# bluenote-1577/sylph

Hardware: AMD Instinct MI355X
Metric: read Gbp/s sketched + genome-comparisons/s profiled, 1 Gbp vs GTDB-R220 (higher is better)
Workload: dtype u64

## Files before the change

sylph_amd/csrc/common.h:

```cpp
#pragma once
#include <hip/hip_runtime.h>

#include <atomic>
#include <cstdarg>
#include <cstdint>
#include <cstdio>
#include <cstdlib>
#include <cstring>
#include <ctime>
#include <map>
#include <mutex>
#include <string>
#include <vector>

#include "../../include/sylph_hip.h"

struct sylph_ctx;

namespace sylph {

void set_error(const char* fmt, ...);

struct HipError { hipError_t e; const char* what; const char* file; int line; };

// ... 134 lines not shown
    sylph::DevBuf scratch[8];
    sylph::DevBuf counters;
    void* pinned = nullptr;
    void read_back(void* dst, const void* dev_src, size_t bytes);
    static constexpr size_t STAGE_BYTES = 32u << 20;
    void* stage[2] = {nullptr, nullptr};
    hipEvent_t stage_ev[2] = {nullptr, nullptr};
    hipStream_t copy_stream = nullptr;
    hipEvent_t copy_ev[2] = {nullptr, nullptr};
    void d2h(void* dst, const void* dev_src, size_t bytes);
    void h2d(void* dev_dst, const void* src, size_t bytes);
};

namespace sylph {

struct ScopedKernelTimer {
    sylph_ctx* ctx;
    hipEvent_t a = nullptr, b = nullptr;
    const char* fam;
    ScopedKernelTimer(sylph_ctx* c, const char* family);
    ~ScopedKernelTimer();
};
void profile_collect(sylph_ctx* ctx);
void ctx_unref(sylph_ctx* ctx);

struct HostPhase {
    sylph_ctx* ctx;
    const char* name;
    double t0 = 0;
    static bool enabled() { static const bool e = getenv("SYLPH_HIP_TRACE") != nullptr; return e; }
    static double now() { timespec ts; clock_gettime(CLOCK_MONOTONIC, &ts); return ts.tv_sec * 1e3 + ts.tv_nsec * 1e-6; }
    HostPhase(sylph_ctx* c, const char* n) : ctx(c), name(n) { if (enabled()) { (void)hipStreamSynchronize(c->stream); t0 = now(); } }
    ~HostPhase() { if (enabled()) { (void)hipStreamSynchronize(ctx->stream); fprintf(stderr, "[sylph_hip] %-28s %8.3f ms\n", name, now() - t0); } }
};

struct DeviceGuard {
    int prev = -1;
    explicit DeviceGuard(int dev) {
        (void)hipGetDevice(&prev);
        if (prev != dev) SY_HIP(hipSetDevice(dev));
        else prev = -1;
    }
    ~DeviceGuard() { if (prev >= 0) (void)hipSetDevice(prev); }
};

void sort_pairs_u64_u32(sylph_ctx* ctx, const uint64_t* kin, uint64_t* kout, const uint32_t* vin, uint32_t* vout,
                        size_t n, int begin_bit, int end_bit);
void sort_pairs_u32_u64(sylph_ctx* ctx, const uint32_t* kin, uint32_t* kout, const uint64_t* vin, uint64_t* vout,
                        size_t n, int begin_bit, int end_bit);
void sort_pairs_u32_u32(sylph_ctx* ctx, const uint32_t* kin, uint32_t* kout, const uint32_t* vin, uint32_t* vout,
                        size_t n, int begin_bit, int end_bit);
constexpr uint32_t SPILL_MAX_TILES = 256;
struct SpillState { uint32_t n_tiles; uint32_t tiles[SPILL_MAX_TILES]; };
struct ReadsState { uint32_t long_record; SpillState spill; };

void sort_keys_u32(sylph_ctx* ctx, const uint32_t* kin, uint32_t* kout, size_t n, int begin_bit, int end_bit);
void sort_keys_u64(sylph_ctx* ctx, const uint64_t* kin, uint64_t* kout, size_t n, int begin_bit, int end_bit);
void exclusive_sum_u32(sylph_ctx* ctx, const uint32_t* in, uint32_t* out, size_t n);
void inclusive_max_u32(sylph_ctx* ctx, const uint32_t* in, uint32_t* out, size_t n);

inline int bit_length(uint64_t v) { int b = 0; while (v) { b++; v >>= 1; } return b; }

}
```

sylph_amd/csrc/reads.hip:

```cpp
#include <cstddef>

#include "common.h"
#include "device_common.h"
#include "sketch_session.h"

namespace sylph {

namespace {

constexpr int RTPB = 256;
constexpr int RT_MIN = 4096, RT_MAX = 65536;
constexpr int RH = 400;
constexpr int RPAD = 32;
constexpr int MASKW = 12;
constexpr int OFFS_256 = 600;
constexpr int RTPB_RAGGED = 512;

template <int K>
struct KC {
    static constexpr uint64_t MASK = (1ull << (2 * K)) - 1;
};

__device__ __forceinline__ uint64_t win64(const uint32_t* sF, uint32_t b) {
    const uint32_t j = b >> 4, ph = (b & 15u) * 2u;
    const uint64_t x = ((uint64_t)sF[j] << 32) | sF[j + 1];
    return (x << ph) | ((uint64_t)sF[j + 2] >> (32u - ph));
}

template <int K>
__device__ __forceinline__ uint64_t revcomp_top(uint64_t x) {
    const uint64_t rev = __brevll(x);
    const uint64_t y = ((rev & 0x5555555555555555ull) << 1) | ((rev >> 1) & 0x5555555555555555ull);
    return (~y) & KC<K>::MASK;
}

__device__ __forceinline__ uint32_t even_fields_to_bytes31(uint32_t w) {
    uint32_t t = w & 0xCCCCCCCCu;
    t = (t | (t << 2)) & 0xF0F0F0F0u;
    return t | (t << 4);
}
__device__ __forceinline__ void evenodd16(uint64_t x, uint32_t& ev, uint32_t& od) {
    const uint32_t hi = (uint32_t)(x >> 32), lo = (uint32_t)x;
    ev = __builtin_amdgcn_perm(even_fields_to_bytes31(hi), even_fields_to_bytes31(lo), 0x07050301u);
    od = __builtin_amdgcn_perm(even_fields_to_bytes31(hi << 2), even_fields_to_bytes31(lo << 2), 0x07050301u);
}

template <int K, int T, int HV>
__device__ __forceinline__ void kmer_step(uint32_t A0, uint32_t A1, uint32_t A2, uint32_t Bm, uint32_t B0, uint32_t B1, uint32_t B2,
                                          uint64_t thr, uint32_t& mask) {
    constexpr int D = 64 - 2 * K;
    uint32_t fhi, flo, rhi, rlo;
    if constexpr (T == 0) { fhi = A0; flo = A1; }
    else { fhi = __builtin_amdgcn_alignbit(A0, A1, 32 - 2 * T); flo = __builtin_amdgcn_alignbit(A1, A2, 32 - 2 * T); }
    constexpr int OFF = 2 * T - D;
    if constexpr (OFF < 0) { rlo = __builtin_amdgcn_alignbit(B0, Bm, OFF + 32); rhi = __builtin_amdgcn_alignbit(B1, B0, OFF + 32); }
    else if constexpr (OFF == 0) { rlo = B0; rhi = B1; }
    else { rlo = __builtin_amdgcn_alignbit(B1, B0, OFF); rhi = __builtin_amdgcn_alignbit(B2, B1, OFF); }
    const uint64_t f = ((uint64_t)fhi << 32) | flo, rc = ((uint64_t)rhi << 32) | rlo;
    const uint64_t canon = (f < rc ? f : rc) >> D;
    if constexpr (HV == 2) {
        const uint32_t u = mm_hash64_gfx950_hi1(canon);
        asm("v_cmp_ge_u32 vcc, %2, %1\n\tv_addc_co_u32 %0, vcc, %0, %0, vcc" : "+v"(mask) : "v"(u), "s"((uint32_t)thr) : "vcc");
    } else {
        const uint64_t h = HV ? mm_hash64_gfx950(canon) : mm_hash64(canon);
        asm("v_cmp_lt_u64 vcc, %1, %2\n\tv_addc_co_u32 %0, vcc, %0, %0, vcc" : "+v"(mask) : "v"(h), "s"(thr) : "vcc");
    }
}
template <int K, int T0, int HV>
__device__ __forceinline__ void kmer_steps8(uint32_t A0, uint32_t A1, uint32_t A2, uint32_t Bm, uint32_t B0, uint32_t B1, uint32_t B2,
                                            uint64_t thr, uint32_t& mask) {
    kmer_step<K, T0 + 0, HV>(A0, A1, A2, Bm, B0, B1, B2, thr, mask);
    kmer_step<K, T0 + 1, HV>(A0, A1, A2, Bm, B0, B1, B2, thr, mask);
    kmer_step<K, T0 + 2, HV>(A0, A1, A2, Bm, B0, B1, B2, thr, mask);
    kmer_step<K, T0 + 3, HV>(A0, A1, A2, Bm, B0, B1, B2, thr, mask);
    kmer_step<K, T0 + 4, HV>(A0, A1, A2, Bm, B0, B1, B2, thr, mask);
    kmer_step<K, T0 + 5, HV>(A0, A1, A2, Bm, B0, B1, B2, thr, mask);
    kmer_step<K, T0 + 6, HV>(A0, A1, A2, Bm, B0, B1, B2, thr, mask);
    kmer_step<K, T0 + 7, HV>(A0, A1, A2, Bm, B0, B1, B2, thr, mask);
}

__global__ __launch_bounds__(256) void block_records_kernel(const uint64_t* __restrict__ off, uint64_t n_rec, uint32_t bias,
                                                            uint32_t rt, uint32_t n_entries, uint32_t* __restrict__ blk_rec,
                                                            uint32_t* __restrict__ count_sentinel, uint32_t* __restrict__ state_words) {
    const uint32_t b = blockIdx.x * blockDim.x + threadIdx.x;
    if (b == 0) { *count_sentinel = 0; state_words[0] = 0; state_words[1] = 0; }
    if (b >= n_entries) return;
    const uint64_t target = (uint64_t)b * rt;
    uint64_t lo = 0, hi = n_rec;
    while (lo < hi) {
        const uint64_t mid = (lo + hi) >> 1;
        if (off[mid] + bias < target) lo = mid + 1; else hi = mid;
    }
    blk_rec[b] = (uint32_t)lo;
}

#ifndef SYLPH_READS_HASH_DEFAULT
#define SYLPH_READS_HASH_DEFAULT 1
#endif
#ifndef SYLPH_READS_WAVES
#define SYLPH_READS_WAVES 5
#endif
template <int K, int HV, int ENC, int TPB>
__global__ __launch_bounds__(TPB) __attribute__((amdgpu_waves_per_eu(TPB == 256 ? SYLPH_READS_WAVES : 6, TPB == 256 ? SYLPH_READS_WAVES : 6))) void reads_kernel(const uint8_t* __restrict__ bases_al, uint32_t bias, uint64_t n_al,
                                                     const uint64_t* __restrict__ off, uint64_t n_rec,
                                                     const uint32_t* __restrict__ blk_rec, uint32_t n_blk, uint32_t it_begin, uint32_t it_end,
                                                     uint32_t rt, uint64_t thr,
                                                     uint32_t cand_slack, int avx2_compat, int paired, int want_markers, uint64_t rec_base,
                                                     uint32_t slot_cap, OccRec* __restrict__ slot_rec,
                                                     uint32_t* __restrict__ slot_key, int key_sh,
                                                     uint32_t* __restrict__ blk_count,
                                                     ReadsState* __restrict__ state, const uint32_t* __restrict__ blk_list,
                                                     uint32_t* __restrict__ spill_slot_of_blk) {
    constexpr int RTPB = TPB, OFFS = TPB == 256 ? OFFS_256 : 2 * TPB + 80;
    extern __shared__ uint32_t sF[];
    __shared__ uint64_t s_off[OFFS + 4];
    const uint32_t n_words = (rt + 2 * RH) / 16 + 3;
    __shared__ uint32_t s_mask[MASKW][RTPB];
    __shared__ uint32_t s_wave[RTPB / 64];
    static_assert((OFFS + 4) >= 2 * RTPB, "the marker arrays alias the staged offsets");
    uint64_t* const s_m0 = s_off;
    uint64_t* const s_m1 = s_off + RTPB;
    __shared__ uint32_t s_first[RTPB + 1], s_rel[RTPB];
    __shared__ uint16_t s_perm[RTPB], s_nh[RTPB];
    const uint32_t tid = threadIdx.x, lane = tid & 63, wave = tid >> 6;
    __shared__ uint32_t s_redo, s_redo_deal;
    const uint64_t thr_loop = HV == 2 ? (uint64_t)((uint32_t)(thr >> 32) + 1u + cand_slack) : thr;
    if (tid == 0) s_redo = 0;
    const uint32_t per_xcd = (n_blk + 7) / 8;
    for (uint32_t it0 = it_begin + blockIdx.x; it0 < it_end; it0 += gridDim.x) {
        const uint32_t it = blk_list ? it0 : (it0 & 7u) * per_xcd + (it0 >> 3);
        if (it >= n_blk) continue;
        const uint32_t blk = blk_list ? blk_list[it] : it;
        const int64_t a0 = (int64_t)blk * rt - RH;
        const bool interior = a0 >= 0 && (uint64_t)(a0 + (int64_t)n_words * 16) <= n_al;
        if (interior) {
            if constexpr (ENC == 0) {
                const uint4* __restrict__ src = reinterpret_cast<const uint4*>(bases_al + a0);
                for (uint32_t ci = tid; ci < n_words; ci += RTPB) sF[ci] = pack16_fwd(src[ci]);
            } else {
                const uint32_t* __restrict__ src = reinterpret_cast<const uint32_t*>(bases_al + (a0 >> 2));
                for (uint32_t ci = tid; ci < n_words; ci += RTPB) sF[ci] = __builtin_amdgcn_perm(0u, src[ci], 0x00010203u);
            }
        } else {
            for (uint32_t ci = tid; ci < n_words; ci += RTPB) {
                const int64_t a = a0 + (int64_t)ci * 16;
                if constexpr (ENC == 0) {
                    uint4 v = make_uint4(0, 0, 0, 0);
                    if (a >= 0 && (uint64_t)a < n_al) v = *reinterpret_cast<const uint4*>(bases_al + a);
                    sF[ci] = pack16_fwd(v);
                } else {
                    uint32_t w = 0;
                    if (a >= 0 && (uint64_t)a < n_al) w = *reinterpret_cast<const uint32_t*>(bases_al + (a >> 2));
                    sF[ci] = __builtin_amdgcn_perm(0u, w, 0x00010203u);
                }
            }
        }
        const uint64_t R0 = blk_rec[blk], R1 = blk_rec[blk + 1];
        const uint64_t w_lo = paired ? (R0 & ~1ull) : R0;
        const uint64_t w_hi = min(R1 + 2, n_rec);
        const bool in_lds = (w_hi - w_lo + 1) <= (uint64_t)(OFFS + 4) && (R1 - R0) <= (uint64_t)RTPB;
        if (in_lds)
            for (uint64_t t = tid; t <= w_hi - w_lo; t += RTPB) s_off[t] = off[w_lo + t];
        __syncthreads();
        uint32_t base_prev = 0;
        const uint64_t out0 = (uint64_t)it * slot_cap;
        for (uint64_t pass = R0; pass < R1; pass += RTPB) {
            const uint64_t r = pass + tid;
            const bool active = r < R1;
            uint64_t start = 0, L = 0, s1 = 0, s2 = 0, e2 = 0;
            if (active) {
                if (in_lds) {
                    start = s_off[r - w_lo];
                    L = s_off[r + 1 - w_lo] - start;
                    if (paired) { const uint64_t r1 = (r & ~1ull) - w_lo; s1 = s_off[r1]; s2 = s_off[r1 + 1]; e2 = s_off[r1 + 2]; }
                } else {
                    start = off[r];
                    L = off[r + 1] - start;
                    if (paired) { const uint64_t r1 = r & ~1ull; s1 = off[r1]; s2 = off[r1 + 1]; e2 = off[r1 + 2]; }
                }
            }
            const bool too_long = active && (L > (uint64_t)RH || (paired && (s2 - s1 > (uint64_t)RH || e2 - s2 > (uint64_t)RH)));
            if (too_long) state->long_record = 1u;
            const uint32_t nh = (active && !too_long) ? (uint32_t)n_hashed_kmers(L, K, avx2_compat, 0) : 0u;
            const uint32_t rel = active ? (uint32_t)((int64_t)(start + bias) - a0) : 0u;
            uint32_t* const s_hist = s_first;
            if (tid < 64) s_hist[tid] = 0;
            s_rel[tid] = rel;
            s_nh[tid] = (uint16_t)nh;
#ifndef SYLPH_READS_ALWAYS_DEAL
            if (tid == 0) s_redo_deal = 0;
            __syncthreads();
            if (__ballot(nh != (uint32_t)s_nh[0]) && lane == 0) s_redo_deal = 1;
            __syncthreads();
            const bool dealt = s_redo_deal != 0;
            const uint32_t bin = 63u - ((nh + 7) >> 3);
            uint32_t hg_max = (nh + 7) >> 3, arrival = 0, hc = 0;
            if (dealt) {
                arrival = atomicAdd(&s_hist[bin], 1u);
                __syncthreads();
                hc = s_hist[lane];
                const uint64_t bins_used = __ballot(hc != 0u);
                hg_max = bins_used ? 63u - (uint32_t)(__ffsll((unsigned long long)bins_used) - 1) : 0u;
            }
#else
            __syncthreads();
            const uint32_t bin = 63u - ((nh + 7) >> 3);
            const uint32_t arrival = atomicAdd(&s_hist[bin], 1u);
            __syncthreads();
            const uint32_t hc = s_hist[lane];
            const bool dealt = s_hist[bin] != (uint32_t)RTPB;
            const uint64_t bins_used = __ballot(hc != 0u);
            const uint32_t hg_max = bins_used ? 63u - (uint32_t)(__ffsll((unsigned long long)bins_used) - 1) : 0u;
#endif
            const uint32_t rows_used = min((uint32_t)MASKW, (hg_max * 8u + 31u) >> 5);
            if (dealt) {
                const uint32_t incl = wave_inclusive_sum(hc);
                s_perm[(uint32_t)__shfl((int)(incl - hc), (int)bin) + arrival] = (uint16_t)tid;
                __syncthreads();
            }
            const uint32_t slot = dealt ? s_perm[tid] : tid;
            const uint32_t rel_h = dealt ? s_rel[slot] : rel, nh_h = dealt ? s_nh[slot] : nh;
            uint32_t nh_max = nh_h;
#pragma unroll
            for (int d = 32; d > 0; d >>= 1) nh_max = max(nh_max, (uint32_t)__shfl_xor((int)nh_max, d));
            if (nh_max) {
                const uint32_t w0 = rel_h >> 4, sh = 32u - (rel_h & 15u) * 2u;
                uint32_t raw = sF[w0], nxt = sF[w0 + 1];
                auto next_word = [&](uint32_t j) {
                    const uint32_t a = (uint32_t)((((uint64_t)raw << 32) | nxt) >> sh);
                    raw = nxt;
                    nxt = sF[w0 + j + 2];
                    return a;
                };
                uint32_t A0 = next_word(0), A1 = next_word(1), A2 = next_word(2);
                uint32_t Bm = 0, B0 = rcword(A0), B1 = rcword(A1), B2 = rcword(A2);
                const uint32_t n_half = (nh_max + 7) >> 3;
// ... 174 lines not shown
__global__ __launch_bounds__(1024) void block_total_kernel(const uint32_t* __restrict__ blk_count, uint32_t n_blk, uint32_t* __restrict__ total) {
    __shared__ uint32_t s[16];
    uint32_t v = 0;
    for (uint32_t i = threadIdx.x; i < n_blk; i += 1024) v += blk_count[i];
#pragma unroll
    for (int d = 32; d > 0; d >>= 1) v += (uint32_t)__shfl_xor((int)v, d);
    if ((threadIdx.x & 63) == 0) s[threadIdx.x >> 6] = v;
    __syncthreads();
    if (threadIdx.x == 0) {
        uint32_t t = 0;
        for (int w = 0; w < 16; w++) t += s[w];
        *total = t;
    }
}

struct SlotMeta {
    uint32_t *blk_rec, *blk_count, *spill_slot, *blk_off;
    ReadsState* state;
    SlotMeta(sylph_sketch* sk, uint32_t n_blk) {
        blk_rec = sk->slot_meta.as<uint32_t>();
        blk_count = blk_rec + (n_blk + 1);
        spill_slot = blk_count + (n_blk + 1);
        blk_off = spill_slot + (n_blk + 1);
        state = reinterpret_cast<ReadsState*>(blk_off + (n_blk + 1));
    }
};

void compact_region(sylph_sketch* sk, uint32_t n_blk, uint32_t slot_cap, uint32_t n, uint32_t spill_cap, const OccRec* spill_rec) {
    sylph_ctx* ctx = sk->ctx;
    SlotMeta m(sk, n_blk);
    exclusive_sum_u32(ctx, m.blk_count, m.blk_off, (size_t)n_blk + 1);
    const uint64_t need = sk->n_occ + n;
    sk->hash.grow_keep(need * 8, sk->n_occ * 8, ctx->stream);
    sk->recs.grow_keep(need * sizeof(OccRec), sk->n_occ * sizeof(OccRec), ctx->stream);
    {
        ScopedKernelTimer t(ctx, "compact");
        hipLaunchKernelGGL(compact_occ_kernel, dim3(std::min<uint32_t>(n_blk, 1u << 16)), dim3(64), 0, ctx->stream,
                           sk->slot_rec.as<OccRec>(), m.blk_count, m.blk_off, n_blk, slot_cap, spill_cap, spill_rec, m.spill_slot,
                           sk->hash.as<uint64_t>() + sk->n_occ, sk->recs.as<OccRec>() + sk->n_occ);
        SY_HIP(hipGetLastError());
    }
    sk->n_occ = need;
}

}

void resolve_deferred_slots(sylph_sketch* sk) {
    if (!sk->pend.live || !sk->pend.deferred) return;
    sylph_ctx* ctx = sk->ctx;
    SlotMeta m(sk, sk->pend.n_blk);
    hipLaunchKernelGGL(block_total_kernel, dim3(1), dim3(1024), 0, ctx->stream, m.blk_count, sk->pend.n_blk, m.blk_off + sk->pend.n_blk);
    uint32_t res[3] = {0, 0, 0};
    ctx->read_back(res, m.blk_off + sk->pend.n_blk, 12);
    if (res[1] || res[2]) { redo_deferred_batch(sk); return; }
    sk->pend.deferred = false;
    sk->pend.n = res[0];
    if (res[0] == 0) sk->pend = PendingSlots{};
}

void flush_pending_slots(sylph_sketch* sk) {
    resolve_deferred_slots(sk);
    if (!sk->pend.live) return;
    compact_region(sk, sk->pend.n_blk, sk->pend.slot_cap, sk->pend.n, 0, nullptr);
    sk->pend = PendingSlots{};
}

bool push_short_reads(sylph_sketch* sk, const uint8_t* d_bases, uint32_t phase, const uint64_t* d_off, uint64_t n_records, uint64_t n_bases,
                      int enc) {
    sylph_ctx* ctx = sk->ctx;
    const uint32_t bias = enc == SYLPH_ENC_2BIT ? (uint32_t)((uintptr_t)d_bases & 15) * 4u + phase : (uint32_t)((uintptr_t)d_bases & 15);
    const uint8_t* bases_al = d_bases - ((uintptr_t)d_bases & 15);
    const uint64_t n_al = n_bases + bias;
    static const int env_ragged_tpb = [] { const char* e = getenv("SYLPH_HIP_READS_RAGGED_TPB"); return e ? atoi(e) : RTPB; }();
    const bool ragged = (n_bases % n_records) != 0;
    const int tpb = (ragged && env_ragged_tpb == RTPB_RAGGED && (uint64_t)RTPB_RAGGED * 93 / 100 * n_bases / n_records <= (uint64_t)RT_MAX) ? RTPB_RAGGED : RTPB;
    const uint64_t target = ragged ? (uint64_t)tpb * 93 / 100 : (uint64_t)tpb;
    uint32_t rt = (uint32_t)std::min<uint64_t>(RT_MAX, std::max<uint64_t>(RT_MIN, target * n_bases / n_records));
    rt = (rt + 15u) & ~15u;
    const uint32_t n_blk = (uint32_t)(n_al / rt) + 1;
    const uint64_t expect = (uint64_t)rt / sk->c;
    const uint32_t spill_cap = rt + RH;
    const uint32_t slot_cap = (uint32_t)std::min<uint64_t>(spill_cap, expect + expect * 3 / 4 + 48);
    const size_t lds_bytes = ((size_t)(rt + 2 * RH) / 16 + 3 + RPAD) * 4;
    const uint64_t thr = UINT64_MAX / (uint64_t)sk->c;
    sk->slot_rec.reserve((size_t)n_blk * slot_cap * sizeof(OccRec));
    sk->slot_key.reserve((size_t)n_blk * slot_cap * 4);
    sk->slot_meta.reserve(((size_t)n_blk + 1) * 4 * 4 + sizeof(ReadsState) + 16);
    SlotMeta m(sk, n_blk);
    static_assert(offsetof(ReadsState, long_record) == 0 && offsetof(ReadsState, spill) == 4 && offsetof(SpillState, n_tiles) == 0,
                  "long_record and spill.n_tiles are the first two words");
    int cus = 256;
    (void)hipDeviceGetAttribute(&cus, hipDeviceAttributeMultiprocessorCount, ctx->device);
    static const int hv_env = getenv("SYLPH_HIP_HASH_VARIANT") ? atoi(getenv("SYLPH_HIP_HASH_VARIANT")) : SYLPH_READS_HASH_DEFAULT;
    const int hv_want = ctx->reads_hash >= 0 ? ctx->reads_hash : hv_env;
    const uint32_t slack = ctx->reads_slack;
    const int hv = (hv_want == 2 && ((thr >> 32) + 1ull + slack) > 0xFFFFFFFFull) ? 1 : hv_want;
    const int key_sh = key_shift(sk->c);
    auto launch = [&](uint32_t n_it, uint32_t it_b, uint32_t it_e, uint32_t cap, OccRec* sr, uint32_t* skey, const uint32_t* list) {
        if (it_e <= it_b) return;
        const uint32_t grid = ctx->reads_wg_per_cu ? (uint32_t)std::min<uint64_t>(it_e - it_b, (uint64_t)cus * ctx->reads_wg_per_cu) : it_e - it_b;
#define SY_LAUNCH_READS_T(KK, HH, EE, TT)                                                                                             \
    hipLaunchKernelGGL((reads_kernel<KK, HH, EE, TT>), dim3(grid), dim3(TT), lds_bytes, ctx->stream, bases_al, bias, n_al, d_off, n_records, \
                       m.blk_rec, n_it, it_b, it_e, rt, thr, slack, sk->avx2_compat, sk->paired, sk->no_dedup ? 0 : 1, sk->rec_base, cap, sr, skey, key_sh,   \
                       m.blk_count, m.state, list, m.spill_slot)
#define SY_LAUNCH_READS(KK, HH, EE) do { if (tpb == RTPB_RAGGED) SY_LAUNCH_READS_T(KK, HH, EE, RTPB_RAGGED); else SY_LAUNCH_READS_T(KK, HH, EE, RTPB); } while (0)
        if (enc == SYLPH_ENC_2BIT) {
            if (sk->k == 31) { if (hv == 2) SY_LAUNCH_READS(31, 2, 1); else SY_LAUNCH_READS(31, 1, 1); }
            else { if (hv == 2) SY_LAUNCH_READS(21, 2, 1); else SY_LAUNCH_READS(21, 1, 1); }
        } else if (sk->k == 31) { if (hv == 2) SY_LAUNCH_READS(31, 2, 0); else if (hv) SY_LAUNCH_READS(31, 1, 0); else SY_LAUNCH_READS(31, 0, 0); }
        else { if (hv == 2) SY_LAUNCH_READS(21, 2, 0); else if (hv) SY_LAUNCH_READS(21, 1, 0); else SY_LAUNCH_READS(21, 0, 0); }
#undef SY_LAUNCH_READS_T
#undef SY_LAUNCH_READS
        SY_HIP(hipGetLastError());
    };
    {
        HostPhase ph(ctx, "push: reads kernel");
        {
            ScopedKernelTimer t(ctx, "annotate");
            hipLaunchKernelGGL(block_records_kernel, dim3(grid_for(n_blk + 1)), dim3(256), 0, ctx->stream, d_off, n_records, bias, rt,
                               n_blk + 1, m.blk_rec, m.blk_count + n_blk, reinterpret_cast<uint32_t*>(m.state));
        }
        ctx->seed_gate();
        {
            const uint32_t n_round = ((n_blk + 7) / 8) * 8;
            uint32_t cut = n_round;
            if (ctx->turn.done && !ctx->turn.recorded && ctx->reads_tail_pct && n_round >= 64)
                cut = (uint32_t)((uint64_t)n_round * (100 - ctx->reads_tail_pct) / 100) & ~7u;
            {
                ScopedKernelTimer t(ctx, "seeds");
                launch(n_blk, 0, cut, slot_cap, sk->slot_rec.as<OccRec>(), sk->slot_key.as<uint32_t>(), nullptr);
            }
            ctx->seed_done();
            if (cut < n_round) {
                ScopedKernelTimer t(ctx, "seeds");
                launch(n_blk, cut, n_round, slot_cap, sk->slot_rec.as<OccRec>(), sk->slot_key.as<uint32_t>(), nullptr);
            }
        }
        const uint64_t n_expect = (n_bases > n_records * (uint64_t)(sk->k - 1) ? n_bases - n_records * (uint64_t)(sk->k - 1) : 0) / sk->c;
        if (sk->borrow_until_finish && sk->n_occ == 0 && sk->rec_base == 0 && ctx->finish_mode == 0 && sk->c >= 2 && n_expect >= 4096 &&
            (uint64_t)n_blk * slot_cap < (1ull << 31)) {
            sk->pend = PendingSlots{};
            sk->pend.live = true;
            sk->pend.deferred = true;
            sk->pend.n_blk = n_blk;
            sk->pend.slot_cap = slot_cap;
            sk->pend.n = n_blk * slot_cap;
            sk->pend.n_expect = (uint32_t)std::min<uint64_t>(n_expect, sk->pend.n);
            sk->pend.bases = d_bases; sk->pend.phase = phase; sk->pend.off = d_off;
            sk->pend.n_records = n_records; sk->pend.n_bases = n_bases; sk->pend.enc = enc;
            if (ctx->profile) ctx->stats["deferred"].launches++;
            return true;
        }
        hipLaunchKernelGGL(block_total_kernel, dim3(1), dim3(1024), 0, ctx->stream, m.blk_count, n_blk, m.blk_off + n_blk);
    }
    uint32_t res[3] = {0, 0, 0};
    SY_HIP(hipMemcpyAsync(ctx->pinned, m.blk_off + n_blk, 12, hipMemcpyDeviceToHost, ctx->stream));
    SY_HIP(hipStreamSynchronize(ctx->stream));
    memcpy(res, ctx->pinned, 12);
    if (!ctx->pending.empty()) profile_collect(ctx);
    if (res[1] || res[2] > SPILL_MAX_TILES) return false;
    const uint32_t n = res[0];
    if (n == 0) return true;
    if (res[2] == 0 && sk->n_occ == 0 && ctx->finish_mode != 1 && sk->c >= 2) {
        sk->pend.live = true;
        sk->pend.n_blk = n_blk;
        sk->pend.slot_cap = slot_cap;
        sk->pend.n = n;
        return true;
    }
    const OccRec* sp_r = nullptr;
    if (res[2]) {
        DevBuf& b_x = ctx->scratch[7];
        b_x.reserve((size_t)res[2] * spill_cap * sizeof(OccRec));
        OccRec* xr = b_x.as<OccRec>();
        ScopedKernelTimer ts(ctx, "seeds_spill");
        ScopedKernelTimer t(ctx, "seeds");
        launch(res[2], 0, res[2], spill_cap, xr, nullptr, m.state->spill.tiles);
        sp_r = xr;
    }
    compact_region(sk, n_blk, slot_cap, n, spill_cap, sp_r);
    return true;
}

}
```

sylph_amd/csrc/replay_lds.hip:

```cpp
#include "common.h"
#include "device_common.h"
#include "sketch_session.h"
#include "partition.h"

namespace sylph {
namespace {

#ifndef SYLPH_REPLAY_TPB
#define SYLPH_REPLAY_TPB 128
#endif
constexpr int CAP_SMALL = 256, RTPB_SMALL = SYLPH_REPLAY_TPB;
constexpr int CAP_MID = 512, RTPB_MID = 256;
constexpr int CAP_LARGE = 1024, RTPB_LARGE = 256;
constexpr int IDX_BITS = 10;
constexpr uint32_t SEG_LIMIT = 96;


struct ReplayArgs {
    const OccRec* recs;
    const uint64_t* hash;
    const uint32_t* perm;
    const uint32_t* boff;
    const uint32_t* p_nv;
    int paired, dedup;
// ... 877 lines not shown
    uint32_t* chunk_rows = mid_list + (B + 2) + ((B & 1u) ? 1 : 0);
    unsigned long long* chunk_removed = reinterpret_cast<unsigned long long*>(chunk_rows + 264);
    FinishTail* d_tail = b_small.as<FinishTail>();
    const uint32_t* d_nv = boff + B;
    const uint32_t n_zero = (B + 2) * 2;
    const int dbg = getenv("SYLPH_REPLAY_STAGE") ? atoi(getenv("SYLPH_REPLAY_STAGE")) : 0;
    const uint32_t cutoff = sk->paired ? 0u : 4u;
    sk->out_k.reserve((size_t)n_cap * 8);
    sk->out_c.reserve((size_t)n_cap * 4);
    ReplayArgs ra{};
    if (plain) ra.hash = sorted_hash;
    else { ra.recs = recs; ra.perm = b_perm.as<uint32_t>(); }
    ra.boff = boff; ra.p_nv = d_nv;
    ra.paired = sk->paired; ra.dedup = sk->dedup_mode(); ra.cutoff = cutoff; ra.bm = bm;
    ra.tmp_k = b_tmpk.as<uint64_t>(); ra.tmp_c = b_tmpc.as<uint32_t>(); ra.n_distinct = n_distinct; ra.removed_b = removed_b;
    ra.overflow = &d_tail->overflow;
    ra.mid_list = mid_list; ra.large_list = large_list; ra.ovf_list = ovf_list; ra.dbg_stage = dbg;
    {
        HostPhase ph(ctx, "finish(bucket): partition + LDS replay + compact");
        {
            ScopedKernelTimer t(ctx, "sort");
            launch_partition(ctx, in, bm, geom, n_tiles, n_all, hist, pairs, boff, b_perm.as<uint32_t>(), sorted_hash, n_distinct, n_zero,
                             b_small.as<uint32_t>(), large_list, ovf_list, mid_list);
        }
        {
            ScopedKernelTimer t(ctx, "replay");
            if (plain) hipLaunchKernelGGL((bucket_count_kernel<CAP_SMALL, RTPB_SMALL>), dim3(B), dim3(RTPB_SMALL), 0, ctx->stream, ra);
            else hipLaunchKernelGGL((bucket_replay_kernel<CAP_SMALL, RTPB_SMALL>), dim3(B), dim3(RTPB_SMALL), 0, ctx->stream, ra);
        }
    }
    auto close_table = [&](int skip_if_listed) {
        const uint32_t ipt = (B + (1u << 18) - 1) >> 18;
        ScopedKernelTimer t(ctx, "replay");
        hipLaunchKernelGGL(table_scan_kernel, dim3((B + SCAN_CHUNK * ipt - 1) / (SCAN_CHUNK * ipt)), dim3(SCAN_CHUNK), 0, ctx->stream, n_distinct,
                           removed_b, B, ipt, d_off, chunk_rows, chunk_removed);
        hipLaunchKernelGGL(table_compact_kernel, dim3(std::min<uint32_t>((B + 3) / 4, 1u << 15)), dim3(256), 0, ctx->stream,
                           b_tmpk.as<uint64_t>(), b_tmpc.as<uint32_t>(), boff, d_off, chunk_rows, chunk_removed, n_distinct, B, ipt,
                           sk->out_k.as<uint64_t>(), sk->out_c.as<uint32_t>(), ovf_list, mid_list, large_list, skip_if_listed,
                           d_tail, deferred ? sk->slot_meta.as<uint32_t>() + (size_t)(sk->pend.n_blk + 1) * 4 : (const uint32_t*)nullptr,
                           sk->a10_state == 1 ? sk->a10_tail.as<uint32_t>() : (const uint32_t*)nullptr, d_nv);
        SY_HIP(hipGetLastError());
    };
    FinishTail host{};
    auto read_tail = [&] {
        SY_HIP(hipMemcpyAsync(ctx->pinned, d_tail, sizeof host, hipMemcpyDeviceToHost, ctx->stream));
        SY_HIP(hipStreamSynchronize(ctx->stream));
        memcpy(&host, ctx->pinned, sizeof host);
        if (!ctx->pending.empty()) profile_collect(ctx);
    };
    close_table(1);
    read_tail();
    if (deferred) {
        if (host.verdict[0] || host.verdict[1]) {
            redo_deferred_batch(sk);
            a10_mark(sk);
            return finish_bucketed(sk);
        }
        sk->pend.deferred = false;
        sk->pend.n = host.n_found;
    }
    if (!a10_verdict(sk, host.a10_words)) return finish_bucketed(sk);
    if (host.overflow) return false;
    if (plain && host.n_ovf) {
        materialise_plain_records(sk);
        return finish_bucketed(sk);
    }
    if (host.n_mid || host.n_large) {
        HostPhase ph(ctx, "finish(bucket): medium / large configurations");
        {
            ScopedKernelTimer t(ctx, "replay");
            if (plain) {
                if (host.n_large)
                    hipLaunchKernelGGL((bucket_count_list_kernel<CAP_LARGE, RTPB_LARGE>), dim3(std::min<uint32_t>(host.n_large, 1536u)),
                                       dim3(RTPB_LARGE), 0, ctx->stream, ra, large_list);
            } else {
                if (host.n_mid)
                    hipLaunchKernelGGL((bucket_replay_list_kernel<CAP_MID, RTPB_MID>), dim3(std::min<uint32_t>(host.n_mid, 1280u)),
                                       dim3(RTPB_MID), 0, ctx->stream, ra, mid_list);
                if (host.n_large)
                    hipLaunchKernelGGL((bucket_replay_list_kernel<CAP_LARGE, RTPB_LARGE>), dim3(std::min<uint32_t>(host.n_large, 512u)),
                                       dim3(RTPB_LARGE), 0, ctx->stream, ra, large_list);
            }
        }
        close_table(0);
        read_tail();
        if (host.overflow) return false;
    }
    unsigned long long removed_extra = 0;
    if (host.n_ovf) {
        if (ctx->finish_mode == 2 || host.n_ovf > 4096) return false;
        HostPhase ph(ctx, "finish(bucket): overflowing buckets through the device-wide path");
        const uint32_t m = host.n_ovf;
        DevBuf b_so(ctx), b_si(ctx), b_sh(ctx), b_sr(ctx), sub_k(ctx), sub_c(ctx);
        b_so.reserve(((size_t)m + 1) * 4);
        hipLaunchKernelGGL(ovf_offsets_kernel, dim3(1), dim3(1024), 0, ctx->stream, ovf_list, boff, b_so.as<uint32_t>());
        uint32_t n_sub = 0;
        ctx->read_back(&n_sub, b_so.as<uint32_t>() + m, 4);
        b_si.reserve((size_t)n_sub * 8);
        b_sh.reserve((size_t)n_sub * 8);
        b_sr.reserve((size_t)n_sub * sizeof(OccRec));
        uint32_t* sub_idx = b_si.as<uint32_t>();
        uint32_t* sub_sorted = sub_idx + n_sub;
        hipLaunchKernelGGL(ovf_indices_kernel, dim3(m), dim3(256), 0, ctx->stream, ovf_list, b_so.as<uint32_t>(), boff,
                           b_perm.as<uint32_t>(), sub_idx);
        sort_keys_u32(ctx, sub_idx, sub_sorted, n_sub, 0, 32);
        {
            ScopedKernelTimer t(ctx, "replay_overflow");
// ... 21 lines not shown
```

sylph_amd/csrc/sketch.hip:

```cpp
#include <algorithm>
#include <unordered_map>

#include "common.h"
#include "device_common.h"
#include "sketch_session.h"

namespace sylph {

bool finish_bucketed(sylph_sketch* sk);
bool push_short_reads(sylph_sketch* sk, const uint8_t* d_bases, uint32_t phase, const uint64_t* d_off, uint64_t n_records, uint64_t n_bases, int enc);

void launch_seeds(sylph_ctx* ctx, const uint8_t* d_bases, uint32_t n_bases, uint32_t c, uint32_t k, uint64_t* d_out_hash,
                  uint32_t* d_out_pos, uint32_t out_cap, uint32_t* d_count);
uint32_t seeds_slot_capacity(uint32_t c);
uint32_t seeds_n_tiles(uint64_t n_bases);
void launch_seeds_slots(sylph_ctx* ctx, const uint8_t* d_bases, uint32_t n_bases, uint32_t c, uint32_t k, uint32_t slot_cap,
                        uint64_t* d_slot_hash, uint32_t* d_slot_pos, uint32_t* d_tile_count, SpillState* d_spill,
                        const uint32_t* d_tile_list, uint32_t n_list, uint32_t* d_spill_slot_of_tile);
uint32_t seeds_tile_bases();
void launch_compact_slots(sylph_ctx* ctx, const uint64_t* d_slot_hash, const uint32_t* d_slot_pos, const uint32_t* d_tile_count,
                          const uint32_t* d_tile_off, uint32_t n_tiles, uint32_t slot_cap, const uint64_t* d_spill_hash,
                          const uint32_t* d_spill_pos, const uint32_t* d_spill_slot_of_tile, uint32_t* d_out_pos,
                          uint64_t* d_out_hash);

// ... 426 lines not shown
        if (n_records) {
            hipLaunchKernelGGL(marker_lengths_kernel, dim3((uint32_t)std::min<uint64_t>(1024, (n_records + 255) / 256)), dim3(256), 0, ctx->stream,
                               d_off, n_records, d_marked);
            SY_HIP(hipGetLastError());
        }
    }
    if (!plain) materialise_plain_records(sk);
    if (short_batch) done = push_short_reads(sk, d_bases, phase, d_off, n_records, n_bases, enc);
    if (!done && enc == SYLPH_ENC_2BIT) {
        sk->batch_ascii.reserve(n_bases + 64);
        if (n_bases)
            hipLaunchKernelGGL(unpack_2bit_kernel, dim3((uint32_t)std::min<uint64_t>((n_bases + 255) / 256, 65536)), dim3(256), 0, ctx->stream,
                               d_bases, phase, n_bases, sk->batch_ascii.as<uint8_t>());
        SY_HIP(hipMemsetAsync(sk->batch_ascii.as<uint8_t>() + n_bases, 0, 64, ctx->stream));
        d_bases = sk->batch_ascii.as<uint8_t>();
    }
    uint32_t* d_count = sk->counters.as<uint32_t>();
    const uint32_t bias = (uint32_t)((uintptr_t)d_bases & 15);
    const uint32_t n = done ? 0 : seeds_sorted_by_pos(ctx, d_bases - bias, n_bases + bias, sk->c, sk->k, d_count);
    if (plain && !sk->no_dedup && !done) {
        uint32_t marked = 0;
        ctx->read_back(&marked, d_marked, 4);
        if (marked) { plain = false; materialise_plain_records(sk); }
    }
    if (n) {
        HostPhase ph(ctx, "push: grow + annotate");
        const uint64_t need = sk->n_occ + n;
        const size_t keep = sk->n_occ * 8;
        sk->hash.grow_keep(need * 8, keep, ctx->stream);
        if (!plain) sk->recs.grow_keep(need * sizeof(OccRec), sk->n_occ * sizeof(OccRec), ctx->stream);
        const uint32_t n_coarse = (uint32_t)(n_bases >> COARSE_SHIFT) + 2;
        ctx->scratch[5].reserve((size_t)n_coarse * 4);
        ScopedKernelTimer t(ctx, "annotate");
        hipLaunchKernelGGL(coarse_index_kernel, dim3(grid_for(n_coarse)), dim3(256), 0, ctx->stream, d_off, n_records, n_coarse,
                           ctx->scratch[5].as<uint32_t>());
        if (plain)
            hipLaunchKernelGGL(annotate_reads_kernel<true>, dim3(grid_for(n)), dim3(256), 0, ctx->stream, d_bases, d_off, n_records,
                               ctx->scratch[2].as<uint32_t>(), ctx->scratch[3].as<uint64_t>(), n, bias, sk->k, sk->avx2_compat,
                               sk->paired, 0, sk->rec_base, ctx->scratch[5].as<uint32_t>(), sk->hash.as<uint64_t>() + sk->n_occ,
                               (OccRec*)nullptr);
        else
            hipLaunchKernelGGL(annotate_reads_kernel<false>, dim3(grid_for(n)), dim3(256), 0, ctx->stream, d_bases, d_off, n_records,
                               ctx->scratch[2].as<uint32_t>(), ctx->scratch[3].as<uint64_t>(), n, bias, sk->k, sk->avx2_compat,
                               sk->paired, sk->no_dedup ? 0 : 1, sk->rec_base, ctx->scratch[5].as<uint32_t>(),
                               sk->hash.as<uint64_t>() + sk->n_occ, sk->recs.as<OccRec>() + sk->n_occ);
        SY_HIP(hipGetLastError());
        if (plain) sk->n_plain = need;
        sk->n_occ = need;
    }
    sk->rec_base += n_records;
    SY_REQUIRE(sk->rec_base <= RID_MASK, "more than 2^42 records in one sample");
}

void redo_deferred_batch(sylph_sketch* sk) {
    const PendingSlots d = sk->pend;
    sk->pend = PendingSlots{};
    sk->a10_state = 0;
    sk->rec_base -= d.n_records;
    if (sk->ctx->profile) sk->ctx->stats["deferred_redo"].launches++;
    const bool borrow = sk->borrow_until_finish;
    sk->borrow_until_finish = false;
    try { process_batch(sk, d.bases, d.phase, d.off, d.n_records, d.n_bases, d.enc); }
    catch (...) { sk->borrow_until_finish = borrow; throw; }
    sk->borrow_until_finish = borrow;
}

static void push_host_batch(sylph_sketch* sk, const uint8_t* bases, const uint64_t* rec_off, uint64_t n_records, int mem, int enc) {
    sylph_ctx* ctx = sk->ctx;
    const bool pinned = mem == SYLPH_MEM_HOST_PINNED;
    const uint64_t bpb = enc == SYLPH_ENC_2BIT ? 4 : 1;
    if (!ctx->copy_stream) {
        SY_HIP(hipStreamCreateWithFlags(&ctx->copy_stream, hipStreamNonBlocking));
        for (int i = 0; i < 2; i++) SY_HIP(hipEventCreateWithFlags(&ctx->copy_ev[i], hipEventDisableTiming));
    }
    if (!pinned) {
        uint8_t dummy = 0;
        ctx->counters.reserve(64);
        ctx->h2d(ctx->counters.as<uint8_t>() + 32, &dummy, 1);
    }
    const uint64_t max_bytes = std::min<uint64_t>(ctx->push_chunk_bytes, pinned ? (1ull << 31) : (24ull << 20));
    const uint64_t max_recs = pinned ? (4ull << 20) : ((sylph_ctx::STAGE_BYTES - (24ull << 20)) / 8 - 2);
    struct Chunk { uint64_t r0, r1, b0, b1; };
    auto next_chunk = [&](uint64_t r0) {
        const uint64_t b0 = rec_off[r0];
        uint64_t hi = std::min(n_records, r0 + max_recs);
        const uint64_t limit = b0 + std::min<uint64_t>(max_bytes * bpb, 1ull << 31) - 8;
        if (rec_off[hi] > limit) hi = (uint64_t)(std::upper_bound(rec_off + r0, rec_off + hi + 1, limit) - rec_off) - 1;
        if (sk->paired) hi -= (hi - r0) & 1;
        if (hi <= r0) hi = std::min(n_records, r0 + (sk->paired ? 2 : 1));
        return Chunk{r0, hi, b0, rec_off[hi]};
    };
    auto enqueue_copy = [&](const Chunk& c, int slot) {
        const uint64_t byte0 = c.b0 / bpb, byte1 = (c.b1 + bpb - 1) / bpb, nb = byte1 - byte0, no = (c.r1 - c.r0 + 1) * 8;
        sk->slot_bases[slot].reserve(nb + 64);
        sk->slot_off[slot].reserve(no * 2);
        const uint8_t* src_b = bases + byte0;
        const uint64_t* src_o = rec_off + c.r0;
        if (!pinned && nb + no + 8 > sylph_ctx::STAGE_BYTES) {
            SY_HIP(hipStreamSynchronize(ctx->copy_stream));
            ctx->h2d(sk->slot_bases[slot].p, src_b, nb);
            SY_HIP(hipMemsetAsync(sk->slot_bases[slot].as<uint8_t>() + nb, 0, 64, ctx->stream));
            ctx->h2d(sk->slot_off[slot].p, src_o, no);
            SY_HIP(hipEventRecord(ctx->copy_ev[slot], ctx->stream));
            return;
        }
        if (!pinned) {
            SY_HIP(hipEventSynchronize(ctx->stage_ev[slot]));
            uint8_t* stg = (uint8_t*)ctx->stage[slot];
            if (nb) memcpy(stg, src_b, nb);
// ... 466 lines not shown
```

sylph_amd/csrc/sketch_session.h:

```cpp
#pragma once
#include <algorithm>

#include "common.h"

namespace sylph {
constexpr uint64_t RID_MARKER_BIT = 1ull << 63;
constexpr uint64_t RID_A10_BIT = 1ull << 62;
constexpr int RID_RANK_SHIFT = 42;
constexpr uint64_t RID_RANK_MAX = (1ull << 20) - 1;
constexpr uint64_t RID_MASK = (1ull << RID_RANK_SHIFT) - 1;
constexpr uint64_t INVALID_HASH = ~0ull;
struct alignas(32) OccRec { uint64_t hash, rid, m0, m1; };
}

namespace sylph {
void flush_pending_slots(sylph_sketch* sk);
inline int key_shift(uint32_t c) { return std::max(0, bit_length(UINT64_MAX / (uint64_t)std::max<uint32_t>(c, 1)) - 32); }
constexpr int DEDUP_EXACT = 0, DEDUP_NONE = 1, DEDUP_FILTER = 2;
void generic_replay(sylph_ctx* ctx, const uint64_t* d_hash, const OccRec* d_recs, uint32_t n_all, bool paired, int dedup,
                    DevBuf& out_k, DevBuf& out_c, uint64_t& n_out, uint64_t& removed_out);
void a10_mark(sylph_sketch* sk);
void a10_settle(sylph_sketch* sk);
bool a10_verdict(sylph_sketch* sk, const uint32_t words[2]);
void materialise_plain_records(sylph_sketch* sk);
}

namespace sylph {
struct PendingSlots {
    bool live = false;
    uint32_t n_blk = 0, slot_cap = 0, n = 0;
    bool deferred = false;
    uint32_t n_expect = 0;
    const uint8_t* bases = nullptr;
    uint32_t phase = 0;
    const uint64_t* off = nullptr;
    uint64_t n_records = 0, n_bases = 0;
    int enc = 0;
};
void resolve_deferred_slots(sylph_sketch* sk);
void redo_deferred_batch(sylph_sketch* sk);
}

struct sylph_sketch {
    sylph_ctx* ctx;
    uint32_t c, k;
    int paired, no_dedup, avx2_compat;
    bool finished = false;
    bool borrow_until_finish = false;
    double dedup_fpr = 0.;
    uint64_t dedup_capacity = 10000000;
    int a10_state = 0;
    int a10_force = 0;
    bool filter_dedup() const { return paired && !no_dedup && dedup_fpr > 0.; }
    int dedup_mode() const { return no_dedup ? sylph::DEDUP_NONE : (filter_dedup() ? sylph::DEDUP_FILTER : sylph::DEDUP_EXACT); }
    uint64_t rec_base = 0;
    uint64_t n_occ = 0;
    uint64_t n_plain = 0;
    sylph::DevBuf hash;
    sylph::DevBuf recs;
    sylph::DevBuf slot_bases[2], slot_off[2];
    sylph::DevBuf slot_rec, slot_key, slot_meta;
    sylph::PendingSlots pend;
    sylph::DevBuf batch_ascii;
    sylph::DevBuf fq_bases, fq_off;
    sylph::DevBuf out_k, out_c;
    uint64_t n_out = 0, dup_removed = 0;
    sylph::DevBuf counters;
    sylph::DevBuf a10_tail;
    explicit sylph_sketch(sylph_ctx* cx)
        : ctx(cx), hash(cx), recs(cx), slot_bases{sylph::DevBuf(cx), sylph::DevBuf(cx)}, slot_off{sylph::DevBuf(cx), sylph::DevBuf(cx)},
          slot_rec(cx), slot_key(cx), slot_meta(cx), batch_ascii(cx), fq_bases(cx), fq_off(cx), out_k(cx), out_c(cx), counters(cx), a10_tail(cx) {}
};
```

Baseline: 1104.

## Add short-read kernel tier with smaller mask width and higher occupancy

Adds a template MASKW parameter to the reads kernel and a short tier (mask width 5 instead of 12) that is chosen when the average record length fits in 5*32 k-mers. The smaller per-thread mask should reduce register pressure, so waves-per-EU is raised to 7 for that variant. If any record exceeds the short-tier capacity, a TIER flag is set, the sketch switches permanently to the full tier and the batch is redone. The long-record flag is now set once per wave with a ballot and atomicOr. The risk is a costly redo whenever a batch holds reads longer than the average suggests.

```diff
diff --git a/sylph_amd/csrc/common.h b/sylph_amd/csrc/common.h
--- a/sylph_amd/csrc/common.h
+++ b/sylph_amd/csrc/common.h
@@ -210,6 +210,7 @@
                         size_t n, int begin_bit, int end_bit);
 constexpr uint32_t SPILL_MAX_TILES = 256;
 struct SpillState { uint32_t n_tiles; uint32_t tiles[SPILL_MAX_TILES]; };
+constexpr uint32_t LONG_RECORD_HALO = 1u, LONG_RECORD_TIER = 2u;
 struct ReadsState { uint32_t long_record; SpillState spill; };
 
 void sort_keys_u32(sylph_ctx* ctx, const uint32_t* kin, uint32_t* kout, size_t n, int begin_bit, int end_bit);
diff --git a/sylph_amd/csrc/reads.hip b/sylph_amd/csrc/reads.hip
--- a/sylph_amd/csrc/reads.hip
+++ b/sylph_amd/csrc/reads.hip
@@ -12,7 +12,8 @@
 constexpr int RT_MIN = 4096, RT_MAX = 65536;
 constexpr int RH = 400;
 constexpr int RPAD = 32;
-constexpr int MASKW = 12;
+constexpr int MASKW_FULL = 12;
+constexpr int MASKW_SHORT = 5;
 constexpr int OFFS_256 = 600;
 constexpr int RTPB_RAGGED = 512;
 
@@ -98,10 +99,11 @@
 #define SYLPH_READS_HASH_DEFAULT 1
 #endif
 #ifndef SYLPH_READS_WAVES
-#define SYLPH_READS_WAVES 5
+#define SYLPH_READS_WAVES 7
 #endif
-template <int K, int HV, int ENC, int TPB>
-__global__ __launch_bounds__(TPB) __attribute__((amdgpu_waves_per_eu(TPB == 256 ? SYLPH_READS_WAVES : 6, TPB == 256 ? SYLPH_READS_WAVES : 6))) void reads_kernel(const uint8_t* __restrict__ bases_al, uint32_t bias, uint64_t n_al,
+constexpr int reads_waves(int tpb, int maskw) { return tpb != 256 ? 6 : (maskw < MASKW_FULL ? SYLPH_READS_WAVES : 5); }
+template <int K, int HV, int ENC, int TPB, int MASKW>
+__global__ __launch_bounds__(TPB) __attribute__((amdgpu_waves_per_eu(reads_waves(TPB, MASKW), reads_waves(TPB, MASKW)))) void reads_kernel(const uint8_t* __restrict__ bases_al, uint32_t bias, uint64_t n_al,
                                                      const uint64_t* __restrict__ off, uint64_t n_rec,
                                                      const uint32_t* __restrict__ blk_rec, uint32_t n_blk, uint32_t it_begin, uint32_t it_end,
                                                      uint32_t rt, uint64_t thr,
@@ -180,8 +182,13 @@
                 }
             }
             const bool too_long = active && (L > (uint64_t)RH || (paired && (s2 - s1 > (uint64_t)RH || e2 - s2 > (uint64_t)RH)));
-            if (too_long) state->long_record = 1u;
-            const uint32_t nh = (active && !too_long) ? (uint32_t)n_hashed_kmers(L, K, avx2_compat, 0) : 0u;
+            if (__ballot(too_long) && lane == 0) atomicOr(&state->long_record, LONG_RECORD_HALO);
+            uint32_t nh = (active && !too_long) ? (uint32_t)n_hashed_kmers(L, K, avx2_compat, 0) : 0u;
+            if constexpr (MASKW < MASKW_FULL) {
+                const bool beyond = nh > (uint32_t)MASKW * 32u;
+                if (__ballot(beyond) && lane == 0) atomicOr(&state->long_record, LONG_RECORD_TIER);
+                if (beyond) nh = 0u;
+            }
             const uint32_t rel = active ? (uint32_t)((int64_t)(start + bias) - a0) : 0u;
             uint32_t* const s_hist = s_first;
             if (tid < 64) s_hist[tid] = 0;
@@ -462,7 +469,7 @@
     hipLaunchKernelGGL(block_total_kernel, dim3(1), dim3(1024), 0, ctx->stream, m.blk_count, sk->pend.n_blk, m.blk_off + sk->pend.n_blk);
     uint32_t res[3] = {0, 0, 0};
     ctx->read_back(res, m.blk_off + sk->pend.n_blk, 12);
-    if (res[1] || res[2]) { redo_deferred_batch(sk); return; }
+    if (res[1] || res[2]) { redo_deferred_batch(sk, res[1]); return; }
     sk->pend.deferred = false;
     sk->pend.n = res[0];
     if (res[0] == 0) sk->pend = PendingSlots{};
@@ -506,14 +513,18 @@
     const uint32_t slack = ctx->reads_slack;
     const int hv = (hv_want == 2 && ((thr >> 32) + 1ull + slack) > 0xFFFFFFFFull) ? 1 : hv_want;
     const int key_sh = key_shift(sk->c);
+    const bool short_tier = !sk->reads_full_tier && tpb == RTPB && hv != 0 && n_bases / n_records <= (uint64_t)(MASKW_SHORT * 32 + sk->k - 1);
     auto launch = [&](uint32_t n_it, uint32_t it_b, uint32_t it_e, uint32_t cap, OccRec* sr, uint32_t* skey, const uint32_t* list) {
         if (it_e <= it_b) return;
         const uint32_t grid = ctx->reads_wg_per_cu ? (uint32_t)std::min<uint64_t>(it_e - it_b, (uint64_t)cus * ctx->reads_wg_per_cu) : it_e - it_b;
-#define SY_LAUNCH_READS_T(KK, HH, EE, TT)                                                                                             \
-    hipLaunchKernelGGL((reads_kernel<KK, HH, EE, TT>), dim3(grid), dim3(TT), lds_bytes, ctx->stream, bases_al, bias, n_al, d_off, n_records, \
+#define SY_LAUNCH_READS_T(KK, HH, EE, TT, MM)                                                                                         \
+    hipLaunchKernelGGL((reads_kernel<KK, HH, EE, TT, MM>), dim3(grid), dim3(TT), lds_bytes, ctx->stream, bases_al, bias, n_al, d_off, n_records, \
                        m.blk_rec, n_it, it_b, it_e, rt, thr, slack, sk->avx2_compat, sk->paired, sk->no_dedup ? 0 : 1, sk->rec_base, cap, sr, skey, key_sh,   \
                        m.blk_count, m.state, list, m.spill_slot)
-#define SY_LAUNCH_READS(KK, HH, EE) do { if (tpb == RTPB_RAGGED) SY_LAUNCH_READS_T(KK, HH, EE, RTPB_RAGGED); else SY_LAUNCH_READS_T(KK, HH, EE, RTPB); } while (0)
+#define SY_LAUNCH_READS(KK, HH, EE) do {                                                                                               \
+        if (tpb == RTPB_RAGGED) SY_LAUNCH_READS_T(KK, HH, EE, RTPB_RAGGED, MASKW_FULL);                                               \
+        else if (short_tier) SY_LAUNCH_READS_T(KK, HH, EE, RTPB, (HH ? MASKW_SHORT : MASKW_FULL));                                    \
+        else SY_LAUNCH_READS_T(KK, HH, EE, RTPB, MASKW_FULL); } while (0)
         if (enc == SYLPH_ENC_2BIT) {
             if (sk->k == 31) { if (hv == 2) SY_LAUNCH_READS(31, 2, 1); else SY_LAUNCH_READS(31, 1, 1); }
             else { if (hv == 2) SY_LAUNCH_READS(21, 2, 1); else SY_LAUNCH_READS(21, 1, 1); }
@@ -523,6 +534,7 @@
 #undef SY_LAUNCH_READS
         SY_HIP(hipGetLastError());
     };
+    if (ctx->profile && short_tier) ctx->stats["short_tier"].launches++;
     {
         HostPhase ph(ctx, "push: reads kernel");
         {
@@ -568,7 +580,13 @@
     SY_HIP(hipStreamSynchronize(ctx->stream));
     memcpy(res, ctx->pinned, 12);
     if (!ctx->pending.empty()) profile_collect(ctx);
-    if (res[1] || res[2] > SPILL_MAX_TILES) return false;
+    if (res[1] & LONG_RECORD_HALO) return false;
+    if (res[1] & LONG_RECORD_TIER) {
+        sk->reads_full_tier = true;
+        if (ctx->profile) ctx->stats["tier_redo"].launches++;
+        return push_short_reads(sk, d_bases, phase, d_off, n_records, n_bases, enc);
+    }
+    if (res[2] > SPILL_MAX_TILES) return false;
     const uint32_t n = res[0];
     if (n == 0) return true;
     if (res[2] == 0 && sk->n_occ == 0 && ctx->finish_mode != 1 && sk->c >= 2) {
diff --git a/sylph_amd/csrc/replay_lds.hip b/sylph_amd/csrc/replay_lds.hip
--- a/sylph_amd/csrc/replay_lds.hip
+++ b/sylph_amd/csrc/replay_lds.hip
@@ -953,7 +953,7 @@
     read_tail();
     if (deferred) {
         if (host.verdict[0] || host.verdict[1]) {
-            redo_deferred_batch(sk);
+            redo_deferred_batch(sk, host.verdict[0]);
             a10_mark(sk);
             return finish_bucketed(sk);
         }
diff --git a/sylph_amd/csrc/sketch.hip b/sylph_amd/csrc/sketch.hip
--- a/sylph_amd/csrc/sketch.hip
+++ b/sylph_amd/csrc/sketch.hip
@@ -502,9 +502,13 @@
     SY_REQUIRE(sk->rec_base <= RID_MASK, "more than 2^42 records in one sample");
 }
 
-void redo_deferred_batch(sylph_sketch* sk) {
+void redo_deferred_batch(sylph_sketch* sk, uint32_t long_record) {
     const PendingSlots d = sk->pend;
     sk->pend = PendingSlots{};
+    if ((long_record & LONG_RECORD_TIER) && !(long_record & LONG_RECORD_HALO)) {
+        sk->reads_full_tier = true;
+        if (sk->ctx->profile) sk->ctx->stats["tier_redo"].launches++;
+    }
     sk->a10_state = 0;
     sk->rec_base -= d.n_records;
     if (sk->ctx->profile) sk->ctx->stats["deferred_redo"].launches++;
diff --git a/sylph_amd/csrc/sketch_session.h b/sylph_amd/csrc/sketch_session.h
--- a/sylph_amd/csrc/sketch_session.h
+++ b/sylph_amd/csrc/sketch_session.h
@@ -38,7 +38,7 @@
     int enc = 0;
 };
 void resolve_deferred_slots(sylph_sketch* sk);
-void redo_deferred_batch(sylph_sketch* sk);
+void redo_deferred_batch(sylph_sketch* sk, uint32_t long_record);
 }
 
 struct sylph_sketch {
@@ -53,6 +53,7 @@
     int a10_force = 0;
     bool filter_dedup() const { return paired && !no_dedup && dedup_fpr > 0.; }
     int dedup_mode() const { return no_dedup ? sylph::DEDUP_NONE : (filter_dedup() ? sylph::DEDUP_FILTER : sylph::DEDUP_EXACT); }
+    bool reads_full_tier = false;
     uint64_t rec_base = 0;
     uint64_t n_occ = 0;
     uint64_t n_plain = 0;
```

After: 1126 (median of 6 runs). 1.02x the previous value.
